# fengpeng-yue/speech-to-speech-translation

Measured on AMD Instinct MI355X. Metric: mel-frames/sec (fwd+bwd+opt) on Fisher-shaped fbank80->mel80, higher is better.
Workload: dtype bf16; 1 GPU; s2st_transformer base 12enc/6dec d512 nfps4 + aux ASR/ST(1x64) + CTC, recipe dropouts, max-tokens=20000 Fisher-shaped batches, update-freq 1; parallelism=dp1

## Files before the change

### include/s2st_hip.h

```cpp
#ifndef S2ST_HIP_H
#define S2ST_HIP_H
#include <stdint.h>
#ifdef __cplusplus
extern "C" {
#endif

#define S2ST_OK 0
#define S2ST_ERR_LAUNCH (-1)
#define S2ST_ERR_SHAPE (-2)
#define S2ST_ERR_WORKSPACE (-3)
#define S2ST_ERR_ARG (-4)
#define S2ST_ERR_COMM (-5)

typedef struct { int64_t ld; int64_t bs; int32_t per; int32_t _pad; } s2st_split;

typedef struct {
  const void* p;
  int32_t kmajor;
  int32_t dtype;
  s2st_split sp;
  int64_t zo, zi;
} s2st_gemm_operand;

#define S2ST_F32 0
// ... 116 lines not shown
int s2st_halo_image_bf16_f32(const uint16_t* x, int64_t ldx, uint16_t* y, int32_t B, int32_t Tout, int32_t Th, int32_t O, int32_t pad, int32_t stride, void* stream);

int s2st_cast_bf16_halo_f32(const float* x, uint16_t* y, int32_t B, int32_t T, int32_t pad, int32_t C, int32_t plain, void* stream);

int s2st_glu_fwd_img_f32(const float* a, uint16_t* img, int32_t B, int32_t T, int32_t pad, int32_t C, void* stream);

int s2st_glu_bwd_twin_f32(const float* a, const float* dy, s2st_split dysp, float* da, s2st_split dasp, int32_t rows, int32_t C, uint16_t* dah, int64_t ldh, void* stream);

int s2st_glu_bwd_img_f32(const float* a, const float* dy, s2st_split dysp, float* da, s2st_split dasp, int32_t B, int32_t Tout, int32_t Th, int32_t pad, int32_t stride, int32_t C, uint16_t* dah, int64_t ldh, uint16_t* img, void* stream);

int s2st_mel_loss_resid_f32(const float* feat, const float* post, const float* eos, const float* tgt, const int32_t* lens, int32_t B, int32_t D, int32_t F, float pos_weight, float c_l1, float c_mse, float c_eos, float* dfeat, float* dpost, float* deos, void* stream);

int s2st_mel_loss_f32(const float* feat, const float* post, const float* eos, const float* tgt, const int32_t* lens, int32_t B, int32_t D, int32_t F, float pos_weight, float* stats, float c_l1, float c_mse, float c_eos, float* dfeat, float* dpost, float* deos, void* stream);

int s2st_ls_ce_f32(const float* logits, const int64_t* target, int32_t rows, int32_t V, int64_t pad, float eps, float* stats, float* dlogits, float gscale, void* stream);

int s2st_log_softmax_rows_f32(const float* x, int64_t ldx, float* y, int64_t ldy, int32_t rows, int32_t V, int32_t log_out, void* stream);

int s2st_ctc_f32(const float* logits, const int64_t* targets, int32_t Lmax, const int32_t* in_lens, const int32_t* tgt_lens, int32_t B, int32_t E, int32_t V, float* lprobs, float* loss_per_utt, float* dlogits, float gscale, float* ws, void* stream);

int s2st_sumsq_f32(const float* x, int64_t n, float* out, void* stream);
int s2st_sumsq_parts_f32(const float* x, int64_t n, float* parts, void* stream);
int64_t s2st_sumsq_parts_count(int64_t n);

int s2st_adam_f32(float* p, float* g, float* m, float* v, int64_t n, const float* sumsq, float gmul, const float* gmul_dev, float max_norm, float lr, float beta1, float beta2, float eps, float wd, int32_t step, float* gnorm_out, void* p_bf16, int32_t* skipped, int32_t sumsq_parts, int32_t zero_grad, void* stream);

int s2st_grad_pack_bf16_f32(const float* g, uint16_t* out, int64_t n, void* stream);
int s2st_exchange_proxy_f32(const float* bucket, float* scratch, int64_t n, int64_t move_bytes, int32_t wgs, float gbps, void* stream);
int s2st_grad_unpack_bf16_f32(const uint16_t* in, float* g, int64_t n, void* stream);

int64_t s2st_ctc_workspace(int32_t B, int32_t E, int32_t Lmax);

typedef struct {
  int32_t enc_layers, dec_layers, enc_dim, dec_dim, enc_ffn, dec_ffn, enc_heads, dec_heads;
  int32_t enc_pre_ln, dec_pre_ln;
  int32_t in_dim, conv_channels, conv_k;
  int32_t out_dim;
  int32_t prenet_layers, prenet_dim, postnet_layers, postnet_dim, postnet_k;
  int32_t tap_asr, tap_st;
  int32_t has_asr, has_st, has_ctc;
  int32_t asr_layers, asr_dim, st_layers, st_dim, src_vocab, tgt_vocab;
  int32_t no_scale_embedding;
  int32_t precise;
  int32_t tap_dec, has_ctc_tgt;
  int32_t text_input, enc_conv_layers, enc_conv_k;
  int32_t n_speakers, spk_frozen;
// ... 85 lines not shown
typedef struct s2st_dropout_site {
  uint64_t seed;
  int32_t kind;
  int32_t ordinal;
  float p;
  int32_t reserved;
  int64_t dims[5];
  char ctx[24];
} s2st_dropout_site;
int s2st_engine_allow_side_stream(s2st_engine* e, int32_t allow);
int s2st_engine_site_log(s2st_engine* e, int32_t on);
int32_t s2st_engine_site_log_get(const s2st_engine* e, s2st_dropout_site* out, int32_t cap);
int s2st_engine_bind_bf16_transposed(s2st_engine* e, uint16_t* params_bf16_t);
int64_t s2st_engine_workspace_floats(s2st_engine* e, const s2st_batch* geometry);
int s2st_engine_forward(s2st_engine* e, const s2st_batch* b, const s2st_outputs* out,
                        float* workspace, int64_t workspace_floats, void* stream);
int s2st_engine_backward(s2st_engine* e, float gscale, int32_t segment, void* stream);
int32_t s2st_engine_num_segments(const s2st_engine* e);
void* s2st_engine_side_stream(const s2st_engine* e);
int32_t s2st_engine_dec_overlap_active(const s2st_engine* e);
int s2st_engine_segment_range(const s2st_engine* e, int32_t i, int64_t* lo, int64_t* hi);
int s2st_engine_adam_overlapped(s2st_engine* e, float* exp_avg, float* exp_avg_sq, const float* sumsq_parts, int32_t n_parts, float gmul, const float* gmul_dev, float max_norm, float lr, float beta1, float beta2, float eps, float wd, int32_t step, float* gnorm_out, int32_t* skipped, int32_t write_bf16, int32_t n_chunks, void* stream);
int s2st_engine_wait_optimizer(s2st_engine* e, void* stream);

int64_t s2st_engine_decode_state_floats(const s2st_engine* e, int32_t B, int32_t E, int32_t max_steps);
int s2st_engine_decode_begin(s2st_engine* e, const s2st_batch* b, const s2st_outputs* out, float* state,
                             int64_t state_floats, int32_t max_steps, float* workspace,
                             int64_t workspace_floats, void* stream);
int s2st_engine_decode_row_map(s2st_engine* e, const int32_t* row_map);
int s2st_engine_decode_step(s2st_engine* e, int32_t step, const float* prev, const int32_t* pos,
                            const int32_t* self_klen ,
                            uint64_t seed, float* feat_out, float* eos_prob, float* attn_out, float* workspace,
                            int64_t workspace_floats, void* stream);

typedef struct {
  int32_t* step;
  uint64_t* seeds;
  float* cur_feat;
  float* cur_eos;
  float* cur_attn;
  float* pe_cur;
} s2st_decode_replay;
int32_t s2st_engine_decode_replay_supported(const s2st_engine* e);
int s2st_engine_decode_replay_begin(s2st_engine* e, const s2st_decode_replay* r, uint64_t seed0, void* stream);
int s2st_engine_decode_step_replay(s2st_engine* e, const s2st_decode_replay* r, const int32_t* self_klen, float* workspace,
                                   int64_t workspace_floats, void* stream);
// ... 137 lines not shown
```

### speech-to-speech-translation_amd/csrc/c_api.cpp

```cpp
#include <hip/hip_ext.h>
#include "s2st_ops.h"

extern "C" {

int s2st_version(void) { return 100; }

int s2st_experimental_build(void) {
#ifdef S2ST_EXPERIMENTAL
  return 1;
#else
  return 0;
#endif
}

int s2st_device_count(void) {
  int n = 0;
  if (hipGetDeviceCount(&n) != hipSuccess) return 0;
  return n;
}

int s2st_exchange_proxy_f32(const float* bucket, float* scratch, int64_t n, int64_t move_bytes, int32_t wgs, float gbps, void* stream) {
  return s2st_exchange_proxy(bucket, scratch, (long)n, (long)move_bytes, wgs, gbps, (hipStream_t)stream);
}
int s2st_grad_pack_bf16_f32(const float* g, uint16_t* out, int64_t n, void* stream) {
// ... 142 lines not shown
  return s2st_glu_bwd_img(a, dy, dysp, da, dasp, B, Tout, Th, pad, stride, C, (hipStream_t)stream, dah, (long)ldh, img);
}

int s2st_mel_loss_resid_f32(const float* feat, const float* post, const float* eos, const float* tgt, const int32_t* lens, int32_t B, int32_t D, int32_t F, float pos_weight, float c_l1, float c_mse, float c_eos, float* dfeat, float* dpost, float* deos, void* stream) {
  return s2st_mel_loss(feat, post, eos, tgt, lens, B, D, F, pos_weight, nullptr, c_l1, c_mse, c_eos, dfeat, dpost, deos, (hipStream_t)stream, nullptr, nullptr, 1);
}

int s2st_mel_loss_f32(const float* feat, const float* post, const float* eos, const float* tgt, const int32_t* lens, int32_t B, int32_t D, int32_t F, float pos_weight, float* stats, float c_l1, float c_mse, float c_eos, float* dfeat, float* dpost, float* deos, void* stream) {
  return s2st_mel_loss(feat, post, eos, tgt, lens, B, D, F, pos_weight, stats, c_l1, c_mse, c_eos, dfeat, dpost, deos, (hipStream_t)stream);
}

int s2st_ls_ce_f32(const float* logits, const int64_t* target, int32_t rows, int32_t V, int64_t pad, float eps, float* stats, float* dlogits, float gscale, void* stream) {
  return s2st_ls_ce(logits, (const long*)target, rows, V, pad, eps, stats, dlogits, gscale, (hipStream_t)stream);
}

int s2st_ctc_f32(const float* logits, const int64_t* targets, int32_t Lmax, const int32_t* in_lens, const int32_t* tgt_lens, int32_t B, int32_t E, int32_t V, float* lprobs, float* loss_per_utt, float* dlogits, float gscale, float* ws, void* stream) {
  return s2st_ctc(logits, (const long*)targets, Lmax, in_lens, tgt_lens, B, E, V, lprobs, loss_per_utt, dlogits, gscale, ws, (hipStream_t)stream);
}

int s2st_sumsq_parts_f32(const float* x, int64_t n, float* parts, void* stream) {
  return s2st_sumsq_parts(x, n, parts, (hipStream_t)stream);
}
int64_t s2st_sumsq_parts_count(int64_t n) { return s2st_sumsq_nparts((long)n); }
int s2st_sumsq_f32(const float* x, int64_t n, float* out, void* stream) {
  return s2st_sumsq(x, n, out, (hipStream_t)stream);
}

int s2st_adam_f32(float* p, float* g, float* m, float* v, int64_t n, const float* sumsq, float gmul, const float* gmul_dev, float max_norm, float lr, float beta1, float beta2, float eps, float wd, int32_t step, float* gnorm_out, void* p_bf16, int32_t* skipped, int32_t sumsq_parts, int32_t zero_grad, void* stream) {
  return s2st_adam(p, g, m, v, n, sumsq, gmul, gmul_dev, max_norm, lr, beta1, beta2, eps, wd, step, gnorm_out, (hipStream_t)stream, (uint16_t*)p_bf16, skipped, sumsq_parts, zero_grad);
}

int64_t s2st_layernorm_bwd_scratch(int32_t rows, int32_t cols) { return (int64_t)s2st_layernorm_bwd_blocks(rows, cols) * 2 * cols; }
int64_t s2st_ctc_workspace(int32_t B, int32_t E, int32_t Lmax) { return s2st_ctc_workspace_floats(B, E, Lmax); }

int s2st_flash_attn_fwd_bf16(const s2st_attn_args* args, void* stream) { return s2st_flash_attn_fwd(args, (hipStream_t)stream); }
int s2st_flash_attn_bwd_bf16(const s2st_attn_args* args, const float* dO, float* dvec_scratch, void* stream) {
  return s2st_flash_attn_bwd(args, dO, dvec_scratch, (hipStream_t)stream, 0);
}

int s2st_argmax_dim1_f32(const float* x, int64_t* idx, int32_t B, int32_t E, int32_t D, void* stream) {
  return s2st_argmax_dim1(x, (long*)idx, B, E, D, (hipStream_t)stream);
}
int s2st_affine_cols_f32(const float* x, const float* scale, const float* shift, float* y, int64_t rows, int32_t C, void* stream) {
  return s2st_affine_cols(x, scale, shift, y, rows, C, (hipStream_t)stream);
}
int s2st_exp_transpose_f32(const float* x, float* y, int32_t T, int32_t C, void* stream) {
// ... 168 lines not shown
```

### speech-to-speech-translation_amd/csrc/engine.cpp

```cpp
#include <cmath>
#include <cstdio>
#include <cstdlib>
#include <cstring>
#include <functional>
#include <string>
#include <vector>

#include "s2st_ops.h"
#include <hip/hip_ext.h>

namespace {

struct PInfo {
  std::string name;
  long off, numel;
  int ndim;
  int shape[4];
  int is_buffer;
};

struct Ten {
  float* d = nullptr;
  float* g = nullptr;
  bf16raw* h = nullptr;
// ... 344 lines not shown
    if (hipStreamCreateWithFlags(&e->chain1_, hipStreamNonBlocking) == hipSuccess &&
        hipEventCreateWithFlags(&e->ev_cfork_, hipEventDisableTiming) == hipSuccess &&
        hipEventCreateWithFlags(&e->ev_cjoin_, hipEventDisableTiming) == hipSuccess &&
        hipEventCreateWithFlags(&e->ev_cside_, hipEventDisableTiming) == hipSuccess)
      e->nchains = 2;
    else { delete e; return S2ST_ERR_LAUNCH; }
  }
  *out = e;
  return 0;
}

void s2st_engine_destroy(s2st_engine* e) {
  if (!e) return;
  if (e->side_) {
    hipStreamSynchronize(e->side_);
    hipStreamDestroy(e->side_);
    hipEventDestroy(e->ev_fork_);
    hipEventDestroy(e->ev_join_);
    if (e->ev_taps_) hipEventDestroy(e->ev_taps_);
    if (e->ev_auxb_) hipEventDestroy(e->ev_auxb_);
    if (e->ev_kv_) hipEventDestroy(e->ev_kv_);
    if (e->ev_head_) hipEventDestroy(e->ev_head_);
    for (hipEvent_t ev : e->adam_ev) hipEventDestroy(ev);
  }
  if (e->chain1_) {
    hipStreamSynchronize(e->chain1_);
    hipStreamDestroy(e->chain1_);
    if (e->ev_cfork_) hipEventDestroy(e->ev_cfork_);
    if (e->ev_cjoin_) hipEventDestroy(e->ev_cjoin_);
    if (e->ev_cside_) hipEventDestroy(e->ev_cside_);
  }
  e->reset_call();
  delete e;
}

int32_t s2st_engine_num_params(const s2st_engine* e) { return (int32_t)e->infos.size(); }

int s2st_engine_param_info(const s2st_engine* e, int32_t i, s2st_param_info* out) {
  if (i < 0 || i >= (int)e->infos.size()) return S2ST_ERR_ARG;
  const PInfo& p = e->infos[i];
  memset(out, 0, sizeof(*out));
  strncpy(out->name, p.name.c_str(), sizeof(out->name) - 1);
  out->offset = p.off;
  out->numel = p.numel;
  out->ndim = p.ndim;
  for (int k = 0; k < 4; ++k) out->shape[k] = p.shape[k];
// ... 94 lines not shown
    for (int s = 0; s < e->n_segments(); ++s) {
      int rc = e->backward_segment(s);
      if (rc) return rc;
    }
    return 0;
  }
  return e->backward_segment(segment);
}

int s2st_engine_adam_overlapped(s2st_engine* e, float* exp_avg, float* exp_avg_sq, const float* sumsq_parts, int32_t n_parts,
                                float gmul, const float* gmul_dev, float max_norm, float lr, float beta1, float beta2, float eps,
                                float wd, int32_t step, float* gnorm_out, int32_t* skipped, int32_t write_bf16, int32_t n_chunks,
                                void* stream) {
  if (!e || !exp_avg || !exp_avg_sq || !sumsq_parts || n_parts <= 0) return S2ST_ERR_ARG;
  return e->adam_overlapped(exp_avg, exp_avg_sq, sumsq_parts, n_parts, gmul, gmul_dev, max_norm, lr, beta1, beta2, eps, wd, step,
                            gnorm_out, skipped, write_bf16, n_chunks, (hipStream_t)stream);
}

int s2st_engine_wait_optimizer(s2st_engine* e, void* stream) {
  if (!e) return S2ST_ERR_ARG;
  e->adam_wait_all((hipStream_t)stream);
  return 0;
}

int32_t s2st_engine_num_segments(const s2st_engine* e) { return e->n_segments(); }

int32_t s2st_engine_dec_overlap_active(const s2st_engine* e) {
  return e ? (e->dec_early_active ? 1 : 0) | (e->tail_bwd_on_side ? 2 : 0) : 0;
}

void* s2st_engine_side_stream(const s2st_engine* e) {
  const_cast<s2st_engine*>(e)->ensure_side();
  return (void*)e->side_;
}

int s2st_engine_segment_range(const s2st_engine* e, int32_t i, int64_t* lo, int64_t* hi) {
  int ns = e->n_segments();
  if (i < 0 || i >= ns) return S2ST_ERR_ARG;
  *lo = e->marks[ns - i - 1].param_off;
  *hi = e->marks[ns - i].param_off;
  return 0;
}

int64_t s2st_engine_decode_state_floats(const s2st_engine* e, int32_t B, int32_t E, int32_t max_steps) {
  const long Cd = e->c.dec_dim, L = e->c.dec_layers;
  return L * 2 * B * (long)max_steps * Cd + L * (long)B * E * 2 * Cd + 64 + ((long)max_steps + 2) * Cd + L * (long)B * E * Cd + 8;
// ... 320 lines not shown
```

### speech-to-speech-translation_amd/csrc/engine_runtime.h

```cpp
  float* alloc(long n, bool zero = false) {
    n = (n + 63) / 64 * 64;
    float* p = nullptr;
    if (ws_top + n > ws_cap) {
      if (!dry) { oom = true; err = S2ST_ERR_WORKSPACE; }
    } else {
      p = ws + ws_top;
    }
    ws_top += n;
    if (ws_top > ws_peak) ws_peak = ws_top;
    if (p && zero && !dry) hipMemsetAsync(p, 0, sizeof(float) * n, st_);
    return p;
  }
  Ten* newT(int rows, int cols, float* ext = nullptr, bool f32 = true) {
    Ten* t = new Ten();
    t->rows = rows; t->cols = cols;
    t->d = ext ? ext : (f32 ? alloc(t->n()) : nullptr);
    tens.push_back(t);
    return t;
  }
  float* gradbuf(Ten* t, bool& acc) {
    if (t->g) { acc = true; return t->g; }
    t->g = alloc(t->n());
    acc = false;
    return t->g;
// ... 30 lines not shown
  char site_ctx[24] = "";
  void set_ctx(const char* fmt, int i = 0) { snprintf(site_ctx, sizeof site_ctx, fmt, i); }
  uint64_t next_seed(int kind, float p, long d0, long d1 = 0, long d2 = 0, long d3 = 0, long d4 = 0) {
    const uint64_t s = seed * 0x100000001B3ULL + (++site) * 0x9E3779B97F4A7C15ULL;
    if (site_log_on) {
      s2st_dropout_site r{};
      r.seed = s; r.kind = kind; r.p = p;
      r.dims[0] = d0; r.dims[1] = d1; r.dims[2] = d2; r.dims[3] = d3; r.dims[4] = d4;
      snprintf(r.ctx, sizeof r.ctx, "%s", site_ctx);
      int ord = 0;
      for (const s2st_dropout_site& q : site_log) ord += (q.kind == kind && !strcmp(q.ctx, r.ctx)) ? 1 : 0;
      r.ordinal = ord;
      site_log.push_back(r);
    }
    return s;
  }
  void mark() { marks.push_back(Mark{tape.size(), param_watermark}); }
  void touch(long off_end) {
    if (off_end > param_watermark) param_watermark = off_end;
    if (adam_pending && st_ != side_) adam_wait_upto(off_end);
  }

  std::vector<hipEvent_t> adam_ev;
  std::vector<long> adam_lo;
  int adam_next = 0;
  bool adam_pending = false;
  void adam_wait_upto(long off_end) {
    if (!live()) return;
    while (adam_next < (int)adam_lo.size() && adam_lo[adam_next] < off_end) {
      hipStreamWaitEvent(st_, adam_ev[adam_next], 0);
      chains_wait(adam_ev[adam_next]);
      ++adam_next;
    }
    if (adam_next >= (int)adam_lo.size()) adam_pending = false;
  }
  int adam_overlapped(float* m, float* v, const float* sumsq, int nparts, float gmul, const float* gmul_dev, float max_norm,
                      float lr, float b1, float b2, float eps, float wd, int step, float* gnorm_out, int* skipped, int use_ph,
                      int nchunks, hipStream_t main) {
    if (!P || !G || n_params <= 0) return S2ST_ERR_ARG;
    if (nchunks < 1) nchunks = 1;
    if (nchunks > 64) nchunks = 64;
    ensure_side();
    hipStream_t saved = st_;
    st_ = main;
    hipStream_t a = side_ ? fork_side() : main;
    st_ = saved;
    while ((int)adam_ev.size() < nchunks) {
      hipEvent_t e;
      if (hipEventCreateWithFlags(&e, hipEventDisableTiming) != hipSuccess) return S2ST_ERR_LAUNCH;
      adam_ev.push_back(e);
    }
    adam_lo.assign(nchunks, 0);
    int rc = 0;
    for (int c2 = 0; c2 < nchunks && !rc; ++c2) {
      const long lo = (n_params * c2 / nchunks) / 64 * 64, hi = c2 + 1 == nchunks ? n_params : (n_params * (c2 + 1) / nchunks) / 64 * 64;
      adam_lo[c2] = lo;
      rc = s2st_adam(P + lo, G + lo, m + lo, v + lo, hi - lo, sumsq, gmul, gmul_dev, max_norm, lr, b1, b2, eps, wd, step,
                     c2 == 0 ? gnorm_out : nullptr, a, (use_ph && PH) ? reinterpret_cast<uint16_t*>(PH) + lo : nullptr,
                     c2 == 0 ? skipped : nullptr, nparts, 1);
      if (side_) hipEventRecord(adam_ev[c2], a);
    }
    adam_next = 0;
    adam_pending = side_ != nullptr && rc == 0;
    return rc;
  }
  void adam_wait_all(hipStream_t stream) {
    if (!adam_pending) return;
    for (int i = adam_next; i < (int)adam_lo.size(); ++i) hipStreamWaitEvent(stream, adam_ev[i], 0);
    adam_next = (int)adam_lo.size();
    adam_pending = false;
  }

  bool group_wgrad = true;
  int group_flush_at = 6;
  std::vector<GemmArgs> pending_wgrad;
  void push_wgrad(const GemmArgs& g) {
    for (const GemmArgs& p : pending_wgrad)
      if (p.C.p == g.C.p) { flush_wgrad(); break; }
    pending_wgrad.push_back(g);
    if ((int)pending_wgrad.size() >= group_flush_at) flush_wgrad();
  }
  void flush_wgrad() {
    if (pending_wgrad.empty()) return;
    if (live()) {
      if (!side_) sync_chains();
      hipStream_t s = (side_ && st_ != side_) ? fork_side() : st_;
#ifdef S2ST_EXPERIMENTAL
      static const bool skip = [] {
        const bool on = s2st_env_on("S2ST_TIMING_SKIP_WGRAD");
        if (on) fprintf(stderr, "[s2st] S2ST_TIMING_SKIP_WGRAD=1: weight-gradient products are SKIPPED -- gradients are WRONG, "
                                "timing experiments only\n");
        return on;
      }();
// ... 25 lines not shown
```

### speech-to-speech-translation_amd/csrc/engine_step.h

```cpp
  bool use_streamk = s2st_env_on("S2ST_GEMM_STREAMK");
  void reset_call() {
    pending_wgrad.clear();
    pending_lnfold = s2st_lnfold_table{};
    s2st_gemm_streamk_unbind_all();
    for (Ten* t : tens) delete t;
    tens.clear();
    tape.clear();
    tape_aware.clear();
    forked_ = false;
    in_region_ = false;
    marks.clear();
    ws_top = 0;
    ws_peak = 0;
    oom = false;
    err = 0;
    site = 0;
    site_log.clear();
    xattn0_idx = 0;
    tail_bwd_on_side = tail_side_ = dec_early_active = false;
    site_ctx[0] = 0;
    param_watermark = 0;
    next_segment = 0;
    skws = nullptr; skws_n = 0; skws_side = nullptr;
  }
// ... 483 lines not shown
    for (size_t i = hi; i-- > lo;) {
      if (aux_bwd_on_side && live()) {
        if (i + 1 == aux_hi_idx && st_ == main_st) { flush_wgrad(); flush_lnfold(); st_ = fork_side(); }
        if (i + 1 == aux_lo_idx && st_ != main_st) { flush_wgrad(); flush_lnfold(); hipEventRecord(ev_auxb_, st_); st_ = main_st; }
        if (i + 1 == aux_wait_idx) wait_traced(main_st, ev_auxb_, "aux decoders' backward (tap gradients)");
      }
      if (tail_bwd_on_side && live()) {
        const bool in_tail = i >= tail_lo_idx && i < tail_hi_idx;
        if (in_tail && st_ == main_st) { st_ = fork_side(); tail_side_ = true; }
        if (!in_tail && tail_side_) { st_ = main_st; tail_side_ = false; }
      }
      if (live() && !(i < tape_aware.size() && tape_aware[i])) sync_chains();
      tape[i]();
      if (err) break;
    }
    flush_wgrad();
    flush_lnfold();
    if (st_ != main_st) {
      if (!tail_side_) hipEventRecord(ev_auxb_, st_);
      st_ = main_st;
    }
    tail_side_ = false;
    if (live()) sync_chains();
    if (seg == ns - 1) join_side();
    return err;
  }
```

### speech-to-speech-translation_amd/csrc/optim.hip

```cpp
#include "s2st_ops.h"
#include "s2st_prof.h"

namespace {

__global__ __launch_bounds__(256) void sumsq_kernel(const float* __restrict__ x, long n,
                                                    float* __restrict__ out, int parts) {
  __shared__ float red[4];
  float a = 0.f;
  long n4 = n >> 2;
  const float4* x4 = reinterpret_cast<const float4*>(x);
  for (long i = (long)blockIdx.x * 256 + threadIdx.x; i < n4; i += (long)gridDim.x * 256) {
    float4 v = x4[i];
    a += v.x * v.x + v.y * v.y + v.z * v.z + v.w * v.w;
  }
  for (long i = (n4 << 2) + (long)blockIdx.x * 256 + threadIdx.x; i < n; i += (long)gridDim.x * 256)
    a += x[i] * x[i];
  a = wave_sum(a);
  if ((threadIdx.x & 63) == 0) red[threadIdx.x >> 6] = a;
  __syncthreads();
  if (threadIdx.x == 0) {
    const float s = red[0] + red[1] + red[2] + red[3];
    if (parts) out[blockIdx.x] = s;
    else atomicAdd(out, s);
  }
}

__device__ __forceinline__ float fold_sumsq_parts(const float* __restrict__ parts, int nparts) {
  __shared__ float red[4];
  float a = 0.f;
  for (int i = threadIdx.x; i < nparts; i += 256) a += parts[i];
  a = wave_sum(a);
  if ((threadIdx.x & 63) == 0) red[threadIdx.x >> 6] = a;
  __syncthreads();
  return (red[0] + red[1]) + (red[2] + red[3]);
}

__device__ __forceinline__ float adam_one(float& g, float& m, float& v, float p, float coef, float b1, float b2,
                                          float eps, float wd_lr, float step_size) {
  g *= coef;
  m = b1 * m + (1.f - b1) * g;
  v = b2 * v + (1.f - b2) * g * g;
  if (wd_lr != 0.f) p -= wd_lr * p;
  return p - step_size * m / (sqrtf(v) + eps);
}
__global__ __launch_bounds__(256) void adam_kernel(float* __restrict__ p, float* __restrict__ g,
// ... 16 lines not shown
  float coef = gmul;
  if (max_norm > 0.f) coef *= fminf(1.f, max_norm / (gn + 1e-6f));
  const float wd_lr = wd * lr;
  for (long i = (long)blockIdx.x * 256 + threadIdx.x; i < n; i += (long)gridDim.x * 256) {
    float gi = __builtin_nontemporal_load(g + i), mi = __builtin_nontemporal_load(m + i), vi = __builtin_nontemporal_load(v + i);
    const float pi = adam_one(gi, mi, vi, __builtin_nontemporal_load(p + i), coef, b1, b2, eps, wd_lr, step_size);
    __builtin_nontemporal_store(zero_grad ? 0.f : gi, g + i);
    __builtin_nontemporal_store(mi, m + i);
    __builtin_nontemporal_store(vi, v + i);
    __builtin_nontemporal_store(pi, p + i);
    if (ph) ph[i] = (uint16_t)(pack_bf16x4(pi, 0.f, 0.f, 0.f).x & 0xffffu);
  }
}

}

static long sumsq_blocks(long n) {
  long blocks = (n / 4 + 255) / 256;
  if (blocks > S2ST_SUMSQ_PARTS) blocks = S2ST_SUMSQ_PARTS;
  return blocks < 1 ? 1 : blocks;
}
int s2st_sumsq(const float* x, long n, float* out, hipStream_t st) {
  if (n <= 0) return 0;
  s2st_launch("sumsq_kernel", 4.0 * n, 0.0, sumsq_kernel, dim3((unsigned)sumsq_blocks(n)), dim3(256), 0, st, x, n, out, 0);
  return hipGetLastError() == hipSuccess ? 0 : S2ST_ERR_LAUNCH;
}
int s2st_sumsq_parts(const float* x, long n, float* parts, hipStream_t st) {
  if (n <= 0) return 0;
  const long blocks = sumsq_blocks(n);
  s2st_launch("sumsq_kernel", 4.0 * n, 0.0, sumsq_kernel, dim3((unsigned)blocks), dim3(256), 0, st, x, n, parts, 1);
  return hipGetLastError() == hipSuccess ? 0 : S2ST_ERR_LAUNCH;
}
long s2st_sumsq_nparts(long n) { return n <= 0 ? 0 : sumsq_blocks(n); }

int s2st_adam(float* p, float* g, float* m, float* v, long n, const float* sumsq, float gmul,
              const float* gmul_dev, float max_norm, float lr, float beta1, float beta2, float eps, float wd, int step,
              float* gnorm_out, hipStream_t st, uint16_t* ph, int* skipped, int sumsq_parts, int zero_grad) {
  if (n <= 0) return 0;
  double bc1 = 1.0 - pow((double)beta1, step), bc2 = 1.0 - pow((double)beta2, step);
  float step_size = (float)((double)lr * sqrt(bc2) / bc1);
  if (((uintptr_t)p | (uintptr_t)g | (uintptr_t)m | (uintptr_t)v) % 16 || (ph && (uintptr_t)ph % 8)) return S2ST_ERR_ARG;
  long blocks = (n + 256 * 4 - 1) / (256 * 4);
  if (blocks > 1024) blocks = 1024;
  s2st_launch("adam_kernel", (32.0 + (ph ? 2.0 : 0.0)) * n, 0.0, adam_kernel, dim3((unsigned)blocks), dim3(256), 0, st, p, g, m,
              v, n, sumsq, gmul, gmul_dev, max_norm, lr, beta1, beta2, eps, wd, step_size, gnorm_out, ph, skipped, sumsq_parts, zero_grad);
  return hipGetLastError() == hipSuccess ? 0 : S2ST_ERR_LAUNCH;
}

namespace {
__global__ __launch_bounds__(256) void grad_pack_bf16_kernel(const float* __restrict__ g, uint16_t* __restrict__ out, long n) {
  const long n4 = n >> 2;
  for (long i = (long)blockIdx.x * 256 + threadIdx.x; i < n4; i += (long)gridDim.x * 256) {
    const float4 v = reinterpret_cast<const float4*>(g)[i];
    reinterpret_cast<uint2*>(out)[i] = pack_bf16x4(v.x, v.y, v.z, v.w);
  }
  for (long i = (n4 << 2) + (long)blockIdx.x * 256 + threadIdx.x; i < n; i += (long)gridDim.x * 256) {
    const uint2 q = pack_bf16x4(g[i], 0.f, 0.f, 0.f);
    out[i] = (uint16_t)(q.x & 0xffffu);
  }
}
__global__ __launch_bounds__(256) void grad_unpack_bf16_kernel(const uint16_t* __restrict__ in, float* __restrict__ g, long n) {
  const long n4 = n >> 2;
  for (long i = (long)blockIdx.x * 256 + threadIdx.x; i < n4; i += (long)gridDim.x * 256) {
    const uint2 q = reinterpret_cast<const uint2*>(in)[i];
    float4 v;
    v.x = __uint_as_float(q.x << 16); v.y = __uint_as_float(q.x & 0xffff0000u);
    v.z = __uint_as_float(q.y << 16); v.w = __uint_as_float(q.y & 0xffff0000u);
    reinterpret_cast<float4*>(g)[i] = v;
  }
// ... 53 lines not shown
```

### speech-to-speech-translation_amd/csrc/s2st_ops.h

```cpp
#pragma once
#include <cstdlib>
static inline const char* s2st_env_str(const char* name) { return getenv(name); }
static inline int s2st_env_int(const char* name, int dflt) { const char* e = getenv(name); return e ? atoi(e) : dflt; }
static inline bool s2st_env_on(const char* name) { return s2st_env_int(name, 0) != 0; }

#include <hip/hip_runtime.h>
#include <stdint.h>
#include "s2st_common.h"

typedef s2st_gemm_operand GemmOperand;
typedef s2st_gemm_out GemmOut;
typedef s2st_gemm_epilogue GemmEpilogue;
typedef s2st_gemm_args GemmArgs;

inline GemmOperand gemm_rowmajor(const float* p, long ld) {
  GemmOperand o;
  o.p = p; o.kmajor = 1; o.dtype = S2ST_F32; o.sp.ld = ld; o.sp.bs = 0; o.sp.per = 0; o.sp._pad = 0;
  o.zo = o.zi = 0;
  return o;
}
inline GemmOperand gemm_colmajor(const float* p, long ld) {
  GemmOperand o = gemm_rowmajor(p, ld);
  o.kmajor = 0;
  return o;
// ... 285 lines not shown
#define S2ST_LOSS_ORDERED_FLOATS (4 * 2048)
struct s2st_loss_parts {
  const float* part[3];
  int nblocks[3];
  int on;
};
int s2st_ls_ce(const float* logits, const long* target, int rows, int V, long pad, float eps,
               float* stats, float* dlogits, float gscale, hipStream_t st, float* ordered = nullptr,
               int* nblocks_out = nullptr);
long s2st_ctc_workspace_floats(int B, int E, int Lmax);
int s2st_ctc(const float* logits, const long* targets, int Lmax, const int* in_lens,
             const int* tgt_lens, int B, int E, int V, float* lprobs, float* loss_per_utt,
             float* dlogits, float gscale, float* ws, hipStream_t st);

int s2st_log_softmax_rows(const float* x, long ldx, float* y, long ldy, int rows, int V, int log_out, hipStream_t st);
int s2st_loss_finalize(float* stats, const float* ctc_per, int B, float nf, float nr, float w_l1,
                       float w_mse, float w_eos, float w_ctc, float w_asr, float w_st, float eps, int Vs,
                       int Vt, float src_ntok, float tgt_ntok, hipStream_t st, const float* ctc_tgt_per = nullptr,
                       float w_ctc_tgt = 0.f, const s2st_loss_parts* parts = nullptr);

int s2st_sumsq(const float* x, long n, float* out , hipStream_t st);
#define S2ST_SUMSQ_PARTS 1024
int s2st_sumsq_parts(const float* x, long n, float* parts, hipStream_t st);
long s2st_sumsq_nparts(long n);
int s2st_adam(float* p, float* g, float* m, float* v, long n, const float* sumsq, float gmul,
              const float* gmul_dev, float max_norm, float lr, float beta1, float beta2, float eps, float wd, int step,
              float* gnorm_out, hipStream_t st, uint16_t* p_bf16 = nullptr ,
              int* skipped = nullptr ,
              int sumsq_parts = 0 ,
              int zero_grad = 0 );
```

### speech-to-speech-translation_amd/runtime/engine.py

```python
from __future__ import annotations

import ctypes as C
import math
import os
from typing import Callable, Dict, List, Optional, Tuple

import torch

from . import binding as bd

PAD = 1


class ModelConfig(C.Structure):
    _fields_ = [(n, C.c_int32) for n in (
        "enc_layers", "dec_layers", "enc_dim", "dec_dim", "enc_ffn", "dec_ffn", "enc_heads",
        "dec_heads", "enc_pre_ln", "dec_pre_ln", "in_dim", "conv_channels", "conv_k", "out_dim",
        "prenet_layers", "prenet_dim", "postnet_layers", "postnet_dim", "postnet_k", "tap_asr",
        "tap_st", "has_asr", "has_st", "has_ctc", "asr_layers", "asr_dim", "st_layers", "st_dim",
        "src_vocab", "tgt_vocab", "no_scale_embedding", "precise", "tap_dec", "has_ctc_tgt", "text_input", "enc_conv_layers", "enc_conv_k",
        "n_speakers", "spk_frozen", "spk_dim")] + [(n, C.c_float) for n in (
        "dropout", "attn_dropout", "act_dropout", "prenet_dropout", "postnet_dropout", "ctc_weight",
        "asr_weight", "st_weight", "w_l1", "w_mse", "w_eos", "bce_pos_weight", "label_smoothing", "ctc_tgt_weight", "enc_dropout")] + \
        [("s2t_mode", C.c_int32)]
# ... 692 lines not shown
        return int(lo.value), int(hi.value)

    def backward(self, gscale: float = 1.0,
                 on_segment: Optional[Callable[[int, int, int], None]] = None):
        if on_segment is None:
            bd.check(self.lib.s2st_engine_backward(self.h, gscale, -1, bd.stream_ptr()), "s2st_engine_backward")
            return
        for i in range(self.num_segments()):
            bd.check(self.lib.s2st_engine_backward(self.h, gscale, i, bd.stream_ptr()), "s2st_engine_backward")
            lo, hi = self.segment_range(i)
            if hi > lo:
                on_segment(i, lo, hi)

    def adam_overlapped(self, exp_avg, exp_avg_sq, sumsq_parts, n_parts, gmul, gmul_dev, max_norm, lr, beta1, beta2, eps, wd,
                        step, gnorm_out, skipped, write_bf16: bool, n_chunks: int = 8):
        f = self.lib.s2st_engine_adam_overlapped
        for t in (exp_avg, exp_avg_sq, sumsq_parts, gnorm_out, skipped):
            bd.require_device(t)
        bd.check(f(self.h, exp_avg.data_ptr(), exp_avg_sq.data_ptr(), sumsq_parts.data_ptr(), int(n_parts), float(gmul),
                   bd.ptr(gmul_dev), float(max_norm), float(lr), float(beta1), float(beta2), float(eps), float(wd), int(step),
                   gnorm_out.data_ptr(), skipped.data_ptr(), 1 if write_bf16 else 0, int(n_chunks), bd.stream_ptr()),
                 "s2st_engine_adam_overlapped")

    def wait_optimizer(self):
        bd.check(self.lib.s2st_engine_wait_optimizer(self.h, bd.stream_ptr()), "s2st_engine_wait_optimizer")

    def zero_grad(self):
        self.grads.zero_()
```

### speech-to-speech-translation_amd/trainer.py

```python
from __future__ import annotations

import os
from typing import Dict, List, Optional

import torch

from .runtime import binding as bd
from .runtime.distributed import GradReducer, all_reduce_scalars, broadcast_, is_dist, world_size
from .runtime.engine import STAT


def inverse_sqrt_lr(num_updates: int, lr: float, warmup_updates: int, warmup_init_lr: float = -1.0) -> float:
    if warmup_init_lr < 0:
        warmup_init_lr = 0.0 if warmup_updates > 0 else lr
    if num_updates < warmup_updates:
        return warmup_init_lr + num_updates * (lr - warmup_init_lr) / warmup_updates
    return lr * warmup_updates ** 0.5 * num_updates ** -0.5


class Trainer:
    def __init__(self, args, task, model, criterion):
        self.args, self.task, self.model, self.criterion = args, task, model, criterion
        self.engine = model.engine
        dev = self.engine.device
# ... 34 lines not shown
        self.engine.wait_optimizer()

    def train_step(self, samples: List[Dict], fast: bool = True, overlap_optimizer: bool = False):
        eng = self.engine
        self.model.train()
        eng.step_seed = (self.seed + self.num_updates) * 1000003
        if not self._grads_clean:
            eng.zero_grad()
        self._grads_clean = False
        sample_size = 0
        logs = []
        hooks = self.reducer.on_segment if self.reducer is not None else None
        for i, sample in enumerate(samples):
            last = i == len(samples) - 1
            seg_hooks = hooks if last else None
            is_dummy = sample is None or len(sample) == 0
            if is_dummy:
                if self._dummy_batch is None:
                    raise RuntimeError("empty batch before any real batch was seen on this rank")
                sample = self._dummy_batch
            elif self._dummy_batch is None:
                self._dummy_batch = sample
            if fast:
                loss, ss, log = self._fast_micro_step(sample, seg_hooks, 0.0 if is_dummy else 1.0)
            else:
                self.criterion.grad_hooks = seg_hooks
                loss, ss, log = self.task.train_step(sample, self.model, self.criterion, None, self.num_updates,
                                                     ignore_grad=is_dummy)
            if not is_dummy:
                sample_size += ss
                logs.append(log)
        self._bump_bn_counters(len(samples))
        gmul_dev = None
        world = world_size()
        if self.reducer is not None:
            self.reducer.finish()
            self.gmul_dev.fill_(float(sample_size))
            all_reduce_scalars(self.gmul_dev)
            self.gmul_dev.reciprocal_()
            gmul_dev, gmul = self.gmul_dev, 1.0
        else:
            if sample_size <= 0:
                raise RuntimeError("no real batch in this update")
            gmul = 1.0 / float(sample_size)
        nparts = self._sumsq_nparts
        bd.call("s2st_sumsq_parts_f32", eng.grads, eng.n_params, self.sumsq_parts)
        lr = self.get_lr()
        import os
        if overlap_optimizer:
            eng.adam_overlapped(self.exp_avg, self.exp_avg_sq, self.sumsq_parts, nparts, gmul, gmul_dev, float(self.clip_norm),
                                lr, self.betas[0], self.betas[1], self.eps, self.wd, self.num_updates + 1, self.gnorm,
                                self.skipped, self._ph() is not None, int(os.environ.get("S2ST_ADAM_CHUNKS", "16")))
        else:
            bd.call("s2st_adam_f32", eng.params, eng.grads, self.exp_avg, self.exp_avg_sq, eng.n_params,
                    self.sumsq_parts, gmul, gmul_dev, float(self.clip_norm), lr, self.betas[0], self.betas[1],
                    self.eps, self.wd, self.num_updates + 1, self.gnorm, self._ph(), self.skipped, nparts, 1)
        self._grads_clean = True
        if self._ph() is not None:
            eng.mark_bf16_fresh()
        self.num_updates += 1
        self.model.set_num_updates(self.num_updates)
        return {"logs": logs, "sample_size": sample_size, "lr": lr, "gnorm": self.gnorm}

    def check_overflow(self):
        self.engine.wait_optimizer()
        n = int(self.skipped.item())
        if n:
            self.skipped.zero_()
            raise FloatingPointError(f"gradients are Nan/Inf in {n} update(s) since the last check "
                                     f"(num_updates={self.num_updates}); those updates were skipped")

    def _fast_micro_step(self, sample, hooks, gscale: float = 1.0):
        fs = getattr(self.criterion, "fast_step", None)
        if fs is not None:
            return fs(self.model, sample, hooks, gscale)
        eng = self.engine
        sample = self.model.front_end_sample(sample)
        out = eng.forward(sample, training=True, want_attn=False, with_loss=True)
        self.criterion.last_outputs = out
        eng.backward(gscale, on_segment=hooks)
        from .criterions.s2st_loss import LazyLog
        c = eng.cfg
        log = LazyLog(out["stats"], {"ntokens": sample["ntokens"], "nsentences": sample["nsentences"],
                                     "sample_size": sample["ntokens"]},
                      getattr(self.criterion, "report_accuracy", False), bool(c.has_asr), bool(c.has_st))
        return out["stats"][STAT["LOSS"]], sample["ntokens"], log

    def _bump_bn_counters(self, n):
        for name, b in self.model.named_buffers():
            if name.endswith("num_batches_tracked"):
                b += n

    def valid_step(self, sample):
        self.engine.wait_optimizer()
        return self.task.valid_step(sample, self.model, self.criterion)
```

Measured before the change: 1.497 million mel-frames/s.

## Overlap gradient-norm reduction with backward tail and add small head Adam chunks

Computes the gradient sum-of-squares inside the backward pass. The part of the parameter range whose gradients are already final is reduced on the main stream while the side stream finishes the last segments, and the rest is reduced after the join. The trainer then skips its separate full sumsq pass. The sumsq kernel becomes a fixed-span, per-block partitioned reduction so partial ranges write deterministic parts. Adam chunking also gains two small head chunks so the first optimizer chunk can start sooner, at the cost of extra events, launches and more complex bookkeeping.

```diff
diff --git a/include/s2st_hip.h b/include/s2st_hip.h
--- a/include/s2st_hip.h
+++ b/include/s2st_hip.h
@@ -162,6 +162,8 @@
 int s2st_sumsq_f32(const float* x, int64_t n, float* out, void* stream);
 int s2st_sumsq_parts_f32(const float* x, int64_t n, float* parts, void* stream);
 int64_t s2st_sumsq_parts_count(int64_t n);
+int s2st_sumsq_parts_range_f32(const float* x, int64_t n, int64_t lo, int64_t hi, float* parts, void* stream);
+int64_t s2st_sumsq_span(int64_t n);
 
 int s2st_adam_f32(float* p, float* g, float* m, float* v, int64_t n, const float* sumsq, float gmul, const float* gmul_dev, float max_norm, float lr, float beta1, float beta2, float eps, float wd, int32_t step, float* gnorm_out, void* p_bf16, int32_t* skipped, int32_t sumsq_parts, int32_t zero_grad, void* stream);
 
@@ -293,6 +295,10 @@
 int s2st_engine_segment_range(const s2st_engine* e, int32_t i, int64_t* lo, int64_t* hi);
 int s2st_engine_adam_overlapped(s2st_engine* e, float* exp_avg, float* exp_avg_sq, const float* sumsq_parts, int32_t n_parts, float gmul, const float* gmul_dev, float max_norm, float lr, float beta1, float beta2, float eps, float wd, int32_t step, float* gnorm_out, int32_t* skipped, int32_t write_bf16, int32_t n_chunks, void* stream);
 int s2st_engine_wait_optimizer(s2st_engine* e, void* stream);
+int32_t s2st_adam_chunk_bounds(int64_t n, int32_t n_chunks, int32_t head, int64_t* lo_out);
+int s2st_engine_bind_grad_norm(s2st_engine* e, float* parts, int32_t n_parts);
+int32_t s2st_engine_grad_norm_done(s2st_engine* e);
+int64_t s2st_engine_grad_norm_split(const s2st_engine* e);
 
 int64_t s2st_engine_decode_state_floats(const s2st_engine* e, int32_t B, int32_t E, int32_t max_steps);
 int s2st_engine_decode_begin(s2st_engine* e, const s2st_batch* b, const s2st_outputs* out, float* state,
diff --git a/speech-to-speech-translation_amd/csrc/c_api.cpp b/speech-to-speech-translation_amd/csrc/c_api.cpp
--- a/speech-to-speech-translation_amd/csrc/c_api.cpp
+++ b/speech-to-speech-translation_amd/csrc/c_api.cpp
@@ -188,6 +188,9 @@
   return s2st_sumsq_parts(x, n, parts, (hipStream_t)stream);
 }
 int64_t s2st_sumsq_parts_count(int64_t n) { return s2st_sumsq_nparts((long)n); }
+int s2st_sumsq_parts_range_f32(const float* x, int64_t n, int64_t lo, int64_t hi, float* parts, void* stream) {
+  return s2st_sumsq_parts_range(x, n, lo, hi, parts, (hipStream_t)stream);
+}
 int s2st_sumsq_f32(const float* x, int64_t n, float* out, void* stream) {
   return s2st_sumsq(x, n, out, (hipStream_t)stream);
 }
diff --git a/speech-to-speech-translation_amd/csrc/engine.cpp b/speech-to-speech-translation_amd/csrc/engine.cpp
--- a/speech-to-speech-translation_amd/csrc/engine.cpp
+++ b/speech-to-speech-translation_amd/csrc/engine.cpp
@@ -390,6 +390,7 @@
     if (e->ev_kv_) hipEventDestroy(e->ev_kv_);
     if (e->ev_head_) hipEventDestroy(e->ev_head_);
     for (hipEvent_t ev : e->adam_ev) hipEventDestroy(ev);
+    for (hipEvent_t ev : e->seg_ev) hipEventDestroy(ev);
   }
   if (e->chain1_) {
     hipStreamSynchronize(e->chain1_);
@@ -530,6 +531,20 @@
   e->adam_wait_all((hipStream_t)stream);
   return 0;
 }
+
+int s2st_engine_bind_grad_norm(s2st_engine* e, float* parts, int32_t n_parts) {
+  if (!e) return S2ST_ERR_ARG;
+  if (parts && ((long)n_parts != s2st_sumsq_nparts(e->n_params) || e->n_params <= 0)) return S2ST_ERR_ARG;
+  e->gn_parts = parts;
+  return S2ST_OK;
+}
+int32_t s2st_engine_grad_norm_done(s2st_engine* e) {
+  if (!e) return 0;
+  const bool d = e->gn_done;
+  e->gn_done = false;
+  return d ? 1 : 0;
+}
+int64_t s2st_engine_grad_norm_split(const s2st_engine* e) { return e ? e->gn_off : 0; }
 
 int32_t s2st_engine_num_segments(const s2st_engine* e) { return e->n_segments(); }
 
diff --git a/speech-to-speech-translation_amd/csrc/engine_runtime.h b/speech-to-speech-translation_amd/csrc/engine_runtime.h
--- a/speech-to-speech-translation_amd/csrc/engine_runtime.h
+++ b/speech-to-speech-translation_amd/csrc/engine_runtime.h
@@ -76,6 +76,7 @@
   }
 
   std::vector<hipEvent_t> adam_ev;
+  bool adam_head = s2st_env_int("S2ST_ADAM_HEAD", 1) != 0;
   std::vector<long> adam_lo;
   int adam_next = 0;
   bool adam_pending = false;
@@ -104,11 +105,12 @@
       if (hipEventCreateWithFlags(&e, hipEventDisableTiming) != hipSuccess) return S2ST_ERR_LAUNCH;
       adam_ev.push_back(e);
     }
-    adam_lo.assign(nchunks, 0);
+    int64_t bounds[64];
+    nchunks = s2st_adam_chunk_bounds(n_params, nchunks, adam_head ? 1 : 0, bounds);
+    adam_lo.assign(bounds, bounds + nchunks);
     int rc = 0;
     for (int c2 = 0; c2 < nchunks && !rc; ++c2) {
-      const long lo = (n_params * c2 / nchunks) / 64 * 64, hi = c2 + 1 == nchunks ? n_params : (n_params * (c2 + 1) / nchunks) / 64 * 64;
-      adam_lo[c2] = lo;
+      const long lo = adam_lo[c2], hi = c2 + 1 == nchunks ? n_params : adam_lo[c2 + 1];
       rc = s2st_adam(P + lo, G + lo, m + lo, v + lo, hi - lo, sumsq, gmul, gmul_dev, max_norm, lr, b1, b2, eps, wd, step,
                      c2 == 0 ? gnorm_out : nullptr, a, (use_ph && PH) ? reinterpret_cast<uint16_t*>(PH) + lo : nullptr,
                      c2 == 0 ? skipped : nullptr, nparts, 1);
@@ -123,6 +125,36 @@
     for (int i = adam_next; i < (int)adam_lo.size(); ++i) hipStreamWaitEvent(stream, adam_ev[i], 0);
     adam_next = (int)adam_lo.size();
     adam_pending = false;
+  }
+
+  float* gn_parts = nullptr;
+  int norm_split = s2st_env_int("S2ST_NORM_SPLIT", 1);
+  bool gn_done = false;
+  long gn_off = 0;
+  std::vector<hipEvent_t> seg_ev;
+  int seg_rec = 0;
+  bool seg_event(int seg) {
+    while ((int)seg_ev.size() <= seg) {
+      hipEvent_t e;
+      if (hipEventCreateWithFlags(&e, hipEventDisableTiming) != hipSuccess) { chk(S2ST_ERR_LAUNCH); return false; }
+      seg_ev.push_back(e);
+    }
+    return true;
+  }
+  void grad_norm_and_join(int ns) {
+    const long L = s2st_sumsq_span(n_params);
+    int d = norm_split < 0 ? 0 : (norm_split > ns - 1 ? ns - 1 : norm_split);
+    if (seg_rec < ns - d) d = 0;
+    long off = d > 0 ? (marks[d].param_off + L - 1) / L * L : n_params;
+    if (off > n_params) off = n_params;
+    if (off < n_params) {
+      if (side_) wait_traced(st_, seg_ev[ns - 1 - d], "gradient norm: second stream up to the split");
+      chk(s2st_sumsq_parts_range(G, n_params, off, n_params, gn_parts, st_));
+    }
+    join_side();
+    chk(s2st_sumsq_parts_range(G, n_params, 0, off, gn_parts, st_));
+    gn_off = off;
+    gn_done = err == 0;
   }
 
   bool group_wgrad = true;
diff --git a/speech-to-speech-translation_amd/csrc/engine_step.h b/speech-to-speech-translation_amd/csrc/engine_step.h
--- a/speech-to-speech-translation_amd/csrc/engine_step.h
+++ b/speech-to-speech-translation_amd/csrc/engine_step.h
@@ -529,6 +529,14 @@
     }
     tail_side_ = false;
     if (live()) sync_chains();
-    if (seg == ns - 1) join_side();
+    if (seg == 0) { seg_rec = 0; gn_done = false; }
+    if (gn_parts && live() && seg == seg_rec && (!side_ || seg_event(seg))) {
+      if (side_) hipEventRecord(seg_ev[seg], side_);
+      seg_rec = seg + 1;
+    }
+    if (seg == ns - 1) {
+      if (gn_parts && live() && G) grad_norm_and_join(ns);
+      else join_side();
+    }
     return err;
   }
diff --git a/speech-to-speech-translation_amd/csrc/optim.hip b/speech-to-speech-translation_amd/csrc/optim.hip
--- a/speech-to-speech-translation_amd/csrc/optim.hip
+++ b/speech-to-speech-translation_amd/csrc/optim.hip
@@ -4,23 +4,42 @@
 namespace {
 
 __global__ __launch_bounds__(256) void sumsq_kernel(const float* __restrict__ x, long n,
-                                                    float* __restrict__ out, int parts) {
+                                                    float* __restrict__ out, long span, long b0) {
   __shared__ float red[4];
   float a = 0.f;
-  long n4 = n >> 2;
-  const float4* x4 = reinterpret_cast<const float4*>(x);
-  for (long i = (long)blockIdx.x * 256 + threadIdx.x; i < n4; i += (long)gridDim.x * 256) {
-    float4 v = x4[i];
-    a += v.x * v.x + v.y * v.y + v.z * v.z + v.w * v.w;
-  }
-  for (long i = (n4 << 2) + (long)blockIdx.x * 256 + threadIdx.x; i < n; i += (long)gridDim.x * 256)
-    a += x[i] * x[i];
+  if (span > 0) {
+    const long lo = (b0 + blockIdx.x) * span, hi = lo + span < n ? lo + span : n;
+    const float4* x4 = reinterpret_cast<const float4*>(x + lo);
+    const long n4 = (hi - lo) >> 2;
+    long i = threadIdx.x;
+    for (; i + 768 < n4; i += 1024) {
+      const float4 v0 = x4[i], v1 = x4[i + 256], v2 = x4[i + 512], v3 = x4[i + 768];
+      a += v0.x * v0.x + v0.y * v0.y + v0.z * v0.z + v0.w * v0.w;
+      a += v1.x * v1.x + v1.y * v1.y + v1.z * v1.z + v1.w * v1.w;
+      a += v2.x * v2.x + v2.y * v2.y + v2.z * v2.z + v2.w * v2.w;
+      a += v3.x * v3.x + v3.y * v3.y + v3.z * v3.z + v3.w * v3.w;
+    }
+    for (; i < n4; i += 256) {
+      const float4 v = x4[i];
+      a += v.x * v.x + v.y * v.y + v.z * v.z + v.w * v.w;
+    }
+    for (long j = lo + (n4 << 2) + threadIdx.x; j < hi; j += 256) a += x[j] * x[j];
+  } else {
+    long n4 = n >> 2;
+    const float4* x4 = reinterpret_cast<const float4*>(x);
+    for (long i = (long)blockIdx.x * 256 + threadIdx.x; i < n4; i += (long)gridDim.x * 256) {
+      float4 v = x4[i];
+      a += v.x * v.x + v.y * v.y + v.z * v.z + v.w * v.w;
+    }
+    for (long i = (n4 << 2) + (long)blockIdx.x * 256 + threadIdx.x; i < n; i += (long)gridDim.x * 256)
+      a += x[i] * x[i];
+  }
   a = wave_sum(a);
   if ((threadIdx.x & 63) == 0) red[threadIdx.x >> 6] = a;
   __syncthreads();
   if (threadIdx.x == 0) {
     const float s = red[0] + red[1] + red[2] + red[3];
-    if (parts) out[blockIdx.x] = s;
+    if (span > 0) out[b0 + blockIdx.x] = s;
     else atomicAdd(out, s);
   }
 }
@@ -83,16 +102,32 @@
 }
 int s2st_sumsq(const float* x, long n, float* out, hipStream_t st) {
   if (n <= 0) return 0;
-  s2st_launch("sumsq_kernel", 4.0 * n, 0.0, sumsq_kernel, dim3((unsigned)sumsq_blocks(n)), dim3(256), 0, st, x, n, out, 0);
+  s2st_launch("sumsq_kernel", 4.0 * n, 0.0, sumsq_kernel, dim3((unsigned)sumsq_blocks(n)), dim3(256), 0, st, x, n, out, 0L, 0L);
+  return hipGetLastError() == hipSuccess ? 0 : S2ST_ERR_LAUNCH;
+}
+int64_t s2st_sumsq_span(int64_t n) {
+  if (n <= 0) return 0;
+  const long per = (n + S2ST_SUMSQ_PARTS - 1) / S2ST_SUMSQ_PARTS;
+  return (per + 1023) / 1024 * 1024;
+}
+long s2st_sumsq_nparts(long n) {
+  if (n <= 0) return 0;
+  const long L = s2st_sumsq_span(n);
+  return (n + L - 1) / L;
+}
+int s2st_sumsq_parts_range(const float* x, long n, long lo, long hi, float* parts, hipStream_t st) {
+  if (n <= 0) return 0;
+  const long L = s2st_sumsq_span(n);
+  if (lo < 0 || hi > n || lo % L || (hi % L && hi != n)) return S2ST_ERR_ARG;
+  if (lo >= hi) return 0;
+  if (!x || !parts || (uintptr_t)x % 16) return S2ST_ERR_ARG;
+  const long b0 = lo / L, blocks = (hi - lo + L - 1) / L;
+  s2st_launch("sumsq_kernel", 4.0 * (hi - lo), 0.0, sumsq_kernel, dim3((unsigned)blocks), dim3(256), 0, st, x, n, parts, L, b0);
   return hipGetLastError() == hipSuccess ? 0 : S2ST_ERR_LAUNCH;
 }
 int s2st_sumsq_parts(const float* x, long n, float* parts, hipStream_t st) {
-  if (n <= 0) return 0;
-  const long blocks = sumsq_blocks(n);
-  s2st_launch("sumsq_kernel", 4.0 * n, 0.0, sumsq_kernel, dim3((unsigned)blocks), dim3(256), 0, st, x, n, parts, 1);
-  return hipGetLastError() == hipSuccess ? 0 : S2ST_ERR_LAUNCH;
-}
-long s2st_sumsq_nparts(long n) { return n <= 0 ? 0 : sumsq_blocks(n); }
+  return s2st_sumsq_parts_range(x, n, 0, n, parts, st);
+}
 
 int s2st_adam(float* p, float* g, float* m, float* v, long n, const float* sumsq, float gmul,
               const float* gmul_dev, float max_norm, float lr, float beta1, float beta2, float eps, float wd, int step,
@@ -106,6 +141,23 @@
   s2st_launch("adam_kernel", (32.0 + (ph ? 2.0 : 0.0)) * n, 0.0, adam_kernel, dim3((unsigned)blocks), dim3(256), 0, st, p, g, m,
               v, n, sumsq, gmul, gmul_dev, max_norm, lr, beta1, beta2, eps, wd, step_size, gnorm_out, ph, skipped, sumsq_parts, zero_grad);
   return hipGetLastError() == hipSuccess ? 0 : S2ST_ERR_LAUNCH;
+}
+
+int32_t s2st_adam_chunk_bounds(int64_t n, int32_t nchunks, int32_t head, int64_t* lo_out) {
+  if (n <= 0 || !lo_out) return 0;
+  if (nchunks < 1) nchunks = 1;
+  if (nchunks > 64) nchunks = 64;
+  const int64_t h0 = 1L << 19, h1 = 1L << 21;
+  const bool use_head = head && nchunks >= 3 && n >= (1L << 22);
+  int32_t cnt = 0;
+  for (int32_t c = 0; c < nchunks; ++c) {
+    int64_t lo;
+    if (!use_head) lo = (n * c / nchunks) / 64 * 64;
+    else if (c < 2) lo = c * h0;
+    else lo = (h0 + h1 + (n - h0 - h1) * (c - 2) / (nchunks - 2)) / 64 * 64;
+    lo_out[cnt++] = lo;
+  }
+  return cnt;
 }
 
 namespace {
diff --git a/speech-to-speech-translation_amd/csrc/s2st_ops.h b/speech-to-speech-translation_amd/csrc/s2st_ops.h
--- a/speech-to-speech-translation_amd/csrc/s2st_ops.h
+++ b/speech-to-speech-translation_amd/csrc/s2st_ops.h
@@ -331,7 +331,10 @@
 int s2st_sumsq(const float* x, long n, float* out , hipStream_t st);
 #define S2ST_SUMSQ_PARTS 1024
 int s2st_sumsq_parts(const float* x, long n, float* parts, hipStream_t st);
+int s2st_sumsq_parts_range(const float* x, long n, long lo, long hi, float* parts, hipStream_t st);
 long s2st_sumsq_nparts(long n);
+extern "C" int64_t s2st_sumsq_span(int64_t n);
+extern "C" int32_t s2st_adam_chunk_bounds(int64_t n, int32_t nchunks, int32_t head, int64_t* lo_out);
 int s2st_adam(float* p, float* g, float* m, float* v, long n, const float* sumsq, float gmul,
               const float* gmul_dev, float max_norm, float lr, float beta1, float beta2, float eps, float wd, int step,
               float* gnorm_out, hipStream_t st, uint16_t* p_bf16 = nullptr ,
diff --git a/speech-to-speech-translation_amd/runtime/engine.py b/speech-to-speech-translation_amd/runtime/engine.py
--- a/speech-to-speech-translation_amd/runtime/engine.py
+++ b/speech-to-speech-translation_amd/runtime/engine.py
@@ -738,6 +738,17 @@
                    gnorm_out.data_ptr(), skipped.data_ptr(), 1 if write_bf16 else 0, int(n_chunks), bd.stream_ptr()),
                  "s2st_engine_adam_overlapped")
 
+    def bind_grad_norm(self, parts: Optional[torch.Tensor], n_parts: int = 0):
+        if parts is not None:
+            bd.require_device(parts)
+        bd.check(self.lib.s2st_engine_bind_grad_norm(self.h, bd.ptr(parts), int(n_parts)), "s2st_engine_bind_grad_norm")
+
+    def grad_norm_done(self) -> bool:
+        return bool(self.lib.s2st_engine_grad_norm_done(self.h))
+
+    def grad_norm_split(self) -> int:
+        return int(self.lib.s2st_engine_grad_norm_split(self.h))
+
     def wait_optimizer(self):
         bd.check(self.lib.s2st_engine_wait_optimizer(self.h, bd.stream_ptr()), "s2st_engine_wait_optimizer")
 
diff --git a/speech-to-speech-translation_amd/trainer.py b/speech-to-speech-translation_amd/trainer.py
--- a/speech-to-speech-translation_amd/trainer.py
+++ b/speech-to-speech-translation_amd/trainer.py
@@ -80,7 +80,8 @@
             elif self._dummy_batch is None:
                 self._dummy_batch = sample
             if fast:
-                loss, ss, log = self._fast_micro_step(sample, seg_hooks, 0.0 if is_dummy else 1.0)
+                loss, ss, log = self._fast_micro_step(sample, seg_hooks, 0.0 if is_dummy else 1.0,
+                                                      norm=last and self.reducer is None)
             else:
                 self.criterion.grad_hooks = seg_hooks
                 loss, ss, log = self.task.train_step(sample, self.model, self.criterion, None, self.num_updates,
@@ -102,7 +103,8 @@
                 raise RuntimeError("no real batch in this update")
             gmul = 1.0 / float(sample_size)
         nparts = self._sumsq_nparts
-        bd.call("s2st_sumsq_parts_f32", eng.grads, eng.n_params, self.sumsq_parts)
+        if not eng.grad_norm_done():
+            bd.call("s2st_sumsq_parts_f32", eng.grads, eng.n_params, self.sumsq_parts)
         lr = self.get_lr()
         import os
         if overlap_optimizer:
@@ -128,7 +130,7 @@
             raise FloatingPointError(f"gradients are Nan/Inf in {n} update(s) since the last check "
                                      f"(num_updates={self.num_updates}); those updates were skipped")
 
-    def _fast_micro_step(self, sample, hooks, gscale: float = 1.0):
+    def _fast_micro_step(self, sample, hooks, gscale: float = 1.0, norm: bool = False):
         fs = getattr(self.criterion, "fast_step", None)
         if fs is not None:
             return fs(self.model, sample, hooks, gscale)
@@ -136,7 +138,13 @@
         sample = self.model.front_end_sample(sample)
         out = eng.forward(sample, training=True, want_attn=False, with_loss=True)
         self.criterion.last_outputs = out
-        eng.backward(gscale, on_segment=hooks)
+        if norm:
+            eng.bind_grad_norm(self.sumsq_parts, self._sumsq_nparts)
+        try:
+            eng.backward(gscale, on_segment=hooks)
+        finally:
+            if norm:
+                eng.bind_grad_norm(None)
         from .criterions.s2st_loss import LazyLog
         c = eng.cfg
         log = LazyLog(out["stats"], {"ntokens": sample["ntokens"], "nsentences": sample["nsentences"],
```

Measured after the change: 1.495 million mel-frames/s. About the same (-0.2%).
